# xinfushe/oclJPEGDecoder

Measured on NVIDIA B200. Metric: MPix/s decoded (1080p 4:2:0 q90 batch), higher is better.
Workload: dtype int32

## Files before the change

ocljpegdecoder_b200/csrc/b2j_internal.h:

```cpp
#ifndef B2J_INTERNAL_H_INCLUDED
#define B2J_INTERNAL_H_INCLUDED

#include <stdint.h>
#include <stddef.h>
#include <vector>

#include "../../include/b2j.h"

namespace b2j {

constexpr int kScanGroups = 4;
constexpr int kScanThreads = 256;
constexpr int kScanChunkBytes = kScanThreads * kScanGroups * 16;
constexpr int kHuffThreads = 128;
constexpr int kSubBytes = 128;
constexpr int kSyncPre = 2;
constexpr int kSyncLanes = kHuffThreads - kSyncPre;
constexpr int kLutBits = 10;
constexpr int kLutBitsDc = 6;
constexpr int kLutHeader = 16;
constexpr int kLutMaxDecode = 12288;
constexpr int kLutMaxEntries = 32768;
constexpr int kWalkBits = 10;
constexpr int kWalkBitsDc = 8;
// ... 26 lines not shown
    uint32_t has_dri;
    uint32_t width, height;
    uint32_t lut_off;
    uint32_t lut_len;
    uint32_t lut_dec_len;
    uint32_t mode;
    uint32_t tot_blks;
    uint32_t ny_blks;
    uint32_t nu_blks;
    uint32_t samp;
    uint32_t yh;
    uint32_t wide_q;
    uint32_t sub_first;
    uint32_t n_sub_max;
    uint32_t scta_first;
};

struct SubRec
{
    uint32_t p;
    uint32_t cz;
    uint32_t nblk;
    int32_t dc[3];
    uint32_t fs;
    uint32_t fc;
};
struct SubMid { uint32_t p, cz, nblk; int32_t dc[3]; uint32_t fs, fc; };
struct SubPre { uint32_t blk; int32_t dc[3]; };
constexpr uint32_t kSubInvalid = 0xFFFFFFFFu;
constexpr uint32_t kSubNone = 0xFFFFFFFFu;
// ... 23 lines not shown
```

ocljpegdecoder_b200/csrc/kernels.cu:

```cuda
#include <cuda.h>
#include <cuda_runtime.h>
#include <stdint.h>

#include "b2j_internal.h"
#include "b2j_math.h"
#include "b2j_sync.h"
#include "kernels.h"

namespace b2j {

__constant__ uint8_t c_zigzag2[64];

static const uint8_t h_zigzag[64] = B2J_ZIGZAG_TABLE;

cudaError_t init_constants()
{
    uint8_t z2[64];
    for (int i = 0; i < 64; i++) z2[i] = (uint8_t)(2 * h_zigzag[i]);
    return cudaMemcpyToSymbol(c_zigzag2, z2, sizeof(z2));
}

struct ScanFlags { uint32_t keep[4], mark[4], term[4]; };

constexpr uint32_t kFlagAll = 0x80808080u;

__device__ __forceinline__ uint32_t eq_ff(uint32_t w)
{
    return ((w & 0x7F7F7F7Fu) + 0x01010101u) & w & kFlagAll;
}
__device__ __forceinline__ void first_n_flags(int n, uint32_t m[4])
{
#pragma unroll
    for (int i = 0; i < 4; i++)
    {
// ... 174 lines not shown
        if (im.has_dri && rank + 1 < im.n_segs)
        {
            seg_start[im.seg_first + rank + 1] = clean_pos + __popc(keep16 & ((1u << j) - 1u));
            const uint32_t wj = j < 4u ? w[0] : (j < 8u ? w[1] : (j < 12u ? w[2] : w[3]));
            const uint32_t bj = (wj >> (8 * (j & 3u))) & 0xFFu;
            if (bj != 0xD0u + (rank & 7u)) atomicOr(&status[img_idx], B2J_ST_RST_MISMATCH);
        }
        rank++;
    }
}

constexpr int kScanMinCtas = 4;
__global__ void __launch_bounds__(kScanThreads, kScanMinCtas)
k_unstuff_fused(const uint8_t *__restrict__ raw, uint8_t *__restrict__ clean, const ImgDev *__restrict__ imgs,
                const uint32_t *__restrict__ chunk_img, uint64_t *__restrict__ chunk_state, uint32_t *__restrict__ clean_len,
                uint32_t *__restrict__ seg_start, int32_t *__restrict__ status)
{
    __shared__ uint32_t s_min;
    __shared__ uint32_t s_warp[kScanThreads / 32];
    __shared__ uint32_t s_base[3];
    __shared__ __align__(16) uint8_t s_out[kScanChunkBytes + 32];
    const uint32_t tid = threadIdx.x, lane = tid & 31, warp = tid >> 5;
    const uint32_t c = blockIdx.x;
    const uint32_t img_idx = chunk_img[c];
    const ImgDev &im = imgs[img_idx];
    const uint32_t k = c - im.chunk_first;
    const uint32_t pos = k * kScanChunkBytes + tid * (16u * kScanGroups);
    ScanThread st;
    st.load_classify(raw + im.raw_off, pos);
    uint32_t term = kNoTerm;
    {
        uint32_t any = 0;
#pragma unroll
        for (int g = 0; g < kScanGroups; g++) any |= st.f[g].term[0] | st.f[g].term[1] | st.f[g].term[2] | st.f[g].term[3];
        if (__syncthreads_or(any != 0u))
        {
            term = block_first_term(st.first_term(), tid, &s_min);
// ... 201 lines not shown
}

__device__ __forceinline__ int32_t extend_sz(uint32_t v, uint32_t size)
{
    const uint32_t u = __funnelshift_l(v, 0u, size);
    const uint32_t neg = (uint32_t)((int32_t)~v >> 31);
    return (int32_t)(u - __funnelshift_l(neg, 0u, size));
}

constexpr uint32_t kZzBytes = 192;
template <bool SYNC>
__global__ void __launch_bounds__(kHuffThreads)
k_huff_decode(const uint8_t *__restrict__ clean, const ImgDev *__restrict__ imgs, const HuffCtaDev *__restrict__ ctas,
              const uint32_t *__restrict__ seg_start, const uint32_t *__restrict__ clean_len,
              const uint16_t *__restrict__ luts, int16_t *__restrict__ coef, int32_t *__restrict__ status,
              const SubRec *__restrict__ recs, const uint4 *__restrict__ cta_base)
{
    extern __shared__ __align__(16) uint8_t smem[];
    uint8_t *s_slots = smem;
    uint8_t *s_zz2 = smem + kHuffThreads * 128;
    uint16_t *s_lut = reinterpret_cast<uint16_t *>(smem + kHuffThreads * 128 + kZzBytes);

    const uint32_t tid = threadIdx.x, lane = tid & 31;
    const HuffCtaDev cta = ctas[blockIdx.x];
    const ImgDev &im = imgs[cta.img];

    {
        const uint4 *src = reinterpret_cast<const uint4 *>(luts + im.lut_off);
        uint4 *dst = reinterpret_cast<uint4 *>(s_lut);
        for (uint32_t k = tid; k < im.lut_dec_len / 8; k += kHuffThreads) dst[k] = __ldg(src + k);
        uint4 *z = reinterpret_cast<uint4 *>(s_slots);
        for (uint32_t k = tid; k < kHuffThreads * 8; k += kHuffThreads) z[k] = make_uint4(0, 0, 0, 0);
        if (tid < 128) s_zz2[tid] = tid < 64 ? c_zigzag2[tid] : (uint8_t)0;
    }
    __syncthreads();

    const uint32_t tot = im.tot_blks, ny = im.ny_blks, nyu = im.ny_blks + im.nu_blks;
    const uint32_t seg = cta.seg_first + tid;
    uint32_t start = 0, end = 0, nblk = 0, blk0 = 0, start_bit = 0, bi = 0;
    int32_t dc0 = 0, dc1 = 0, dc2 = 0;
    int32_t err = 0;
    bool check_end = false, active, decodable;
    if (!SYNC)
    {
        active = seg < im.n_segs;
        if (active)
        {
            start = seg_start[im.seg_first + seg];
            const uint32_t mcu0 = seg * im.restart_interval;
            const uint32_t nmcu = min(im.restart_interval, im.mcu_count - mcu0);
            nblk = nmcu * tot;
            blk0 = im.blk_first + mcu0 * tot;
            if (seg + 1 < im.n_segs) { end = seg_start[im.seg_first + seg + 1]; check_end = (end != kSegInvalid); }
            if (!check_end) end = clean_len[cta.img];
        }
        decodable = active && start != kSegInvalid;
// ... 24 lines not shown
            for (int w = 0; w < kHuffThreads / 32; w++)
                if (w < (int)(tid >> 5)) { const uint4 t = s_wtot[w]; acc.x += t.x; acc.y += t.y; acc.z += t.z; acc.w += t.w; }
            pre.blk = acc.x + ib - rec.nblk;
            pre.dc[0] = (int32_t)acc.y + i0 - rec.dc[0]; pre.dc[1] = (int32_t)acc.z + i1 - rec.dc[1]; pre.dc[2] = (int32_t)acc.w + i2 - rec.dc[2];
        }
        if (active)
        {
            if (rec.fs != kSubNone && pre.blk < im.blk_count)
            {
                nblk = min(rec.nblk, im.blk_count - pre.blk);
                blk0 = im.blk_first + pre.blk;
                start_bit = rec.fs;
                bi = rec.fc;
                dc0 = pre.dc[0]; dc1 = pre.dc[1]; dc2 = pre.dc[2];
            }
            if (seg + 1 == n_sub && pre.blk + rec.nblk < im.blk_count) err |= B2J_ST_OVERRUN;
            end = clean_len[cta.img];
        }
        decodable = active && nblk > 0;
        {
            uint32_t *s_hist = reinterpret_cast<uint32_t *>(s_slots);
            uint32_t *s_wsum = s_hist + 640;
            uint32_t *s_desc = s_hist + 648;
            const uint32_t key = decodable ? bi * 64u + (63u - min(nblk, 63u)) : 639u;
            const uint32_t within = atomicAdd(&s_hist[key], 1u);
            __syncthreads();
            uint32_t h[5], sum = 0;
#pragma unroll
            for (int k = 0; k < 5; k++) { h[k] = s_hist[tid * 5u + k]; sum += h[k]; }
            uint32_t inc = sum;
#pragma unroll
            for (int o = 1; o < 32; o <<= 1)
            {
// ... 98 lines not shown
            {
                uint4 *sp = reinterpret_cast<uint4 *>(s_slots + warp_slot0 + j * 128u + ((ch ^ (j & 7u)) << 4));
                const uint4 v = *sp;
                *sp = make_uint4(0, 0, 0, 0);
                *reinterpret_cast<uint4 *>(coef + (size_t)dst * 64 + ch * 8) = v;
            }
        }
        __syncwarp();
        if (!SYNC && !dead)
        {
            const uint32_t nw_now = br.words_fetched();
            if (nw_now * 4u > seg_bytes + 16u) { err |= B2J_ST_OVERRUN; dead = true; }
        }
        bi = (bi + 1 == tot) ? 0u : bi + 1;
    }

    if (decodable && !dead)
    {
        const uint32_t nw = br.words_fetched();
        const uint64_t bits = (uint64_t)nw * 32u + br.bitpos - bit0;
        const uint64_t used = (bits + 7u) >> 3;
        const uint64_t avail = (uint64_t)end - start;
        if (used > avail) err |= B2J_ST_OVERRUN;
        else if (!SYNC && check_end && used != avail) err |= B2J_ST_SEGMENT_END;
    }
    if (err) atomicOr(&status[cta.img], err);
}

struct DevLut
{
// ... 86 lines not shown
        *chunk_state_k = make_uint4(sh.entry_used[kSyncPre].x, sh.entry_used[kSyncPre].y, sh.cur[last].p, sh.cur[last].cz);
    }
    __syncthreads();
}

__device__ __forceinline__ void sync_stage_lut(uint16_t *s_lut, const uint16_t *__restrict__ luts, const ImgDev &im)
{
    const uint4 *src = reinterpret_cast<const uint4 *>(luts + im.lut_off + im.lut_dec_len);
    uint4 *dst = reinterpret_cast<uint4 *>(s_lut);
    for (uint32_t k = threadIdx.x; k < (im.lut_len - im.lut_dec_len) / 8; k += kHuffThreads) dst[k] = __ldg(src + k);
}

__global__ void __launch_bounds__(kHuffThreads)
k_sync_chunks(const uint8_t *__restrict__ clean, const ImgDev *__restrict__ imgs, const HuffCtaDev *__restrict__ ctas,
              const uint32_t *__restrict__ clean_len, const uint16_t *__restrict__ luts, SubRec *__restrict__ recs,
              uint4 *__restrict__ chunk_state, uint4 *__restrict__ cta_tot, uint32_t *__restrict__ stats, uint32_t use_pre)
{
    extern __shared__ __align__(16) uint8_t smem[];
    __shared__ uint4 s_wtot[kHuffThreads / 32];
    __shared__ __align__(16) WalkCtab s_ctab[16];
    SyncShared &sh = *reinterpret_cast<SyncShared *>(smem);
    uint16_t *s_lut = reinterpret_cast<uint16_t *>(smem + kSyncSharedBytes);
    const HuffCtaDev cta = ctas[blockIdx.x];
    const ImgDev &im = imgs[cta.img];
    const uint32_t bits = clean_len[cta.img] * 8u;
    const uint32_t n_sub = (bits + kSubBytes * 8 - 1) / (kSubBytes * 8);
    if (cta.seg_first >= n_sub)
    {
        if (threadIdx.x == 0) { cta_tot[blockIdx.x] = make_uint4(0u, 0u, 0u, 0u); chunk_state[blockIdx.x] = make_uint4(0u, 0u, 0u, 0u); }
        return;
    }
    sync_stage_lut(s_lut, luts, im);
    __syncthreads();
    uint32_t sm_lut;
    asm volatile("mov.u32 %0, %1;" : "=r"(sm_lut) : "r"(smem_addr(smem) + kSyncSharedBytes));
    DevWalk wk;
    wk.init(clean + im.raw_off, sm_lut, luts + im.lut_off, s_ctab, im);
    __syncthreads();
    SyncChunk ch;
    ch.first = cta.seg_first; ch.n_sub = n_sub; ch.bits = bits;
    const bool pre = use_pre != 0u && cta.seg_first != 0u;
    ch.first_lane = pre ? (cta.seg_first >= (uint32_t)kSyncPre ? 0u : (uint32_t)kSyncPre - cta.seg_first) : (uint32_t)kSyncPre;
    ch.forced = cta.seg_first == 0u;
    ch.forced_entry = make_uint2(0u, 0u);
    sync_run_chunk(wk, sh, ch, recs + im.sub_first, chunk_state + blockIdx.x, cta_tot + blockIdx.x, stats, s_wtot);
}

// ... 539 lines not shown
    if (tid < n_mcus)
    {
        const uint32_t gm = d.mcu_first + tid;
        const uint32_t my = gm / mcu_count_w;
        sd.mcu_xy[tid] = make_uint2(gm - my * mcu_count_w, my);
    }
    if (tid == 0)
    {
        sd.pix = pix + pix_off;
        sd.width = width; sd.height = height;
        sd.mode = d.info & 0xFFu; sd.n_mcus = n_mcus;
        sd.samp = samp;
    }
}

template <bool NARROWQ>
__device__ __forceinline__ TileDev tile_load(TileSmem &sm, const CUtensorMap *tmap, const ImgDev *__restrict__ imgs, const TileDev *__restrict__ tiles,
                                             const uint16_t *__restrict__ qtabs, uint8_t *__restrict__ pix, int32_t *__restrict__ status)
{
    const uint32_t tid = threadIdx.x;
    const TileDev d = tiles[blockIdx.x];
    if (tid == 0)
    {
        mbar_init(&sm.bar, 1);
        asm volatile("fence.mbarrier_init.release.cluster;" ::: "memory");
        mbar_expect_tx(&sm.bar, kTileBlocks * 128);
        tma_load_2d(sm.tile, tmap, 0, (int)d.row_first, &sm.bar);
    }
    side_stage<NARROWQ>(sm.side, imgs, qtabs, d, pix);
    __syncthreads();
    uint32_t spins = 0;
    while (!mbar_try_wait(&sm.bar, 0))
    {
        if (++spins > (1u << 22)) { if (tid == 0) atomicOr(&status[d.img], B2J_ST_INTERNAL); break; }
    }
    return d;
}

constexpr int kIdctMinCtas = 5;
constexpr int kTileColour = 0, kTileGray = 1, kTileGeneric = 2;
template <bool NARROWQ, int FMT, int KIND>
__global__ void __launch_bounds__(kTileBlocks, kIdctMinCtas)
k_idct_csc(const __grid_constant__ CUtensorMap tmap, const ImgDev *__restrict__ imgs, const TileDev *__restrict__ tiles,
           const uint16_t *__restrict__ qtabs, uint8_t *__restrict__ pix, int32_t *__restrict__ status)
{
    TileSmem &sm = *tile_smem();
    const uint32_t tid = threadIdx.x;
    tile_load<NARROWQ>(sm, &tmap, imgs, tiles, qtabs, pix, status);
    if (KIND == kTileGray)
    {
        idct_phase<0, 0, NARROWQ>(sm.tile, sm.side);
        __syncthreads();
        csc_gray<FMT>(sm.tile, sm.side, tid);
    }
    else if (KIND == kTileGeneric)
    {
        idct_phase<-1, -1, NARROWQ>(sm.tile, sm.side);
        __syncthreads();
        csc_generic<FMT>(sm.tile, sm.side, tid);
    }
    else
    {
        idct_dispatch<NARROWQ>(sm.tile, sm.side);
// ... 142 lines not shown
    }
#pragma unroll
    for (int r = 0; r < 2; r++)
    {
        int64_t d[8], o[2];
#pragma unroll
        for (int c = 0; c < 8; c++) d[c] = ((kUsed >> c) & 1u) ? ws[r][c] : 0;
        red2_1d<13 + 2 + 3 + 2>(d, o);
        *reinterpret_cast<uint16_t *>(dst + (size_t)r * pitch) = (uint16_t)(islow_limit(o[0]) | islow_limit(o[1]) << 8);
    }
}

template <uint32_t MINS>
__global__ void __launch_bounds__(kTileBlocks)
k_idct_libjpeg(const __grid_constant__ CUtensorMap tmap, const ImgDev *__restrict__ imgs, const TileDev *__restrict__ tiles,
               const uint16_t *__restrict__ qtabs, uint8_t *__restrict__ samples, int32_t *__restrict__ status)
{
    TileSmem &sm = *tile_smem();
    const uint32_t tid = threadIdx.x;
    const TileDev d = tile_load<false>(sm, &tmap, imgs, tiles, qtabs, samples, status);
    const ImgDev *im = imgs + d.img;
    const uint32_t sp = sm.side.samp, n = sm.side.n_mcus;
    const uint32_t yh = sp & 15u, yv = (sp >> 4) & 15u, uh = (sp >> 8) & 15u, uv = (sp >> 12) & 15u, vh = (sp >> 16) & 15u, vv = (sp >> 20) & 15u;
    const uint32_t ny = yh * yv, nu = uh * uv, tot = ny + nu + vh * vv;
    if (tid >= n * tot) return;
    const uint32_t comp = (tid >= n * ny ? 1u : 0u) + (tid >= n * (ny + nu) ? 1u : 0u);
    const uint32_t before = (comp > 0 ? ny : 0u) + (comp > 1 ? nu : 0u);
    const uint32_t nc = comp == 0 ? ny : (comp == 1 ? nu : vh * vv);
    const uint32_t j = tid - n * before, m = j / nc, k = j % nc;
    const uint32_t h = comp == 0 ? yh : (comp == 1 ? uh : vh), v = comp == 0 ? yv : (comp == 1 ? uv : vv);
    const uint32_t ss = dct_size(h, v, yh, yv, MINS);
    const uint32_t mcu_count = __ldg(&im->mcu_count), mcw = __ldg(&im->mcu_count_w), blk_first = __ldg(&im->blk_first);
    const size_t pitch = (size_t)mcw * h * ss;
    const uint2 mxy = sm.side.mcu_xy[m];
    uint8_t *dst = samples + 64ull * ((size_t)blk_first + (size_t)mcu_count * before) + (size_t)((mxy.y * v + k / h) * ss) * pitch +
// ... 159 lines not shown

size_t huff_smem_bytes(uint32_t max_lut_len) { return (size_t)kHuffThreads * 128 + kZzBytes + (size_t)max_lut_len * 2; }

cudaError_t configure_kernels(uint32_t max_lut_len)
{
    const int hb = (int)huff_smem_bytes(kLutMaxDecode);
    cudaError_t e = cudaFuncSetAttribute(k_huff_decode<false>, cudaFuncAttributeMaxDynamicSharedMemorySize, hb);
    if (e != cudaSuccess) return e;
    e = cudaFuncSetAttribute(k_huff_decode<true>, cudaFuncAttributeMaxDynamicSharedMemorySize, hb);
    if (e != cudaSuccess) return e;
    e = cudaFuncSetAttribute(k_sync_chunks, cudaFuncAttributeMaxDynamicSharedMemorySize, (int)(kSyncSharedBytes + max_lut_len * 2));
    if (e != cudaSuccess) return e;
    return cudaFuncSetAttribute(k_sync_sweep, cudaFuncAttributeMaxDynamicSharedMemorySize, (int)(kSyncSharedBytes + max_lut_len * 2));
}

void launch_prepass(const DecodeArgs &a, cudaStream_t s)
{
    if (a.n_chunks == 0) return;
    k_unstuff_fused<<<a.n_chunks, kScanThreads, 0, s>>>(a.raw, a.clean, a.imgs, a.chunk_img, a.chunk_state, a.clean_len, a.seg_start, a.status);
}

void launch_huffman(const DecodeArgs &a, cudaStream_t s)
{
    if (a.n_huff_ctas == 0) return;
    k_huff_decode<false><<<a.n_huff_ctas, kHuffThreads, huff_smem_bytes(a.max_lut_dec_len), s>>>(a.clean, a.imgs, a.huff_ctas, a.seg_start, a.clean_len,
                                                                                                a.luts, a.coef, a.status, nullptr, nullptr);
}

void launch_huffman_sync(const DecodeArgs &a, cudaStream_t s)
{
    const uint32_t n = a.n_sync_ctas, ni = a.n_sync_imgs;
    if (n == 0 || ni == 0) return;
    const size_t sync_bytes = kSyncSharedBytes + (size_t)a.max_lut_walk_len * 2;
    k_sync_chunks<<<n, kHuffThreads, sync_bytes, s>>>(a.clean, a.imgs, a.sync_ctas, a.clean_len, a.luts, a.recs, a.sync_chunk_state, a.sync_cta_base,
                                                      a.sync_stats, a.sync_use_pre ? 1u : 0u);
    k_sync_sweep<<<ni, kHuffThreads, sync_bytes, s>>>(a.clean, a.imgs, a.sync_imgs, a.clean_len, a.luts, a.recs, a.sync_chunk_state, a.sync_cta_base,
                                                     a.sync_stats);
    k_sync_cta_scan<<<ni, 32, 0, s>>>(a.imgs, a.sync_imgs, a.sync_cta_base);
    k_huff_decode<true><<<n, kHuffThreads, huff_smem_bytes(a.max_lut_dec_len), s>>>(a.clean, a.imgs, a.sync_ctas, a.seg_start, a.clean_len, a.luts,
                                                                                    a.coef, a.status, a.recs, a.sync_cta_base);
}

template <int FMT, int KIND>
static void launch_idct_kind(const DecodeArgs &a, uint32_t first, uint32_t count, cudaStream_t s)
{
    if (count == 0) return;
    const auto kernel = a.any_wide_q ? k_idct_csc<false, FMT, KIND> : k_idct_csc<true, FMT, KIND>;
    kernel<<<count, kTileBlocks, kTileSmemBytes, s>>>(*a.tmap, a.imgs, a.tiles + first, a.qtabs, a.pixels, a.status);
}

template <int FMT>
static void launch_idct_format(const DecodeArgs &a, cudaStream_t s)
{
    launch_idct_kind<FMT, kTileColour>(a, 0, a.gray_tile0, s);
    launch_idct_kind<FMT, kTileGray>(a, a.gray_tile0, a.generic_tile0 - a.gray_tile0, s);
    launch_idct_kind<FMT, kTileGeneric>(a, a.generic_tile0, a.n_tiles - a.generic_tile0, s);
}

template <int FMT, uint32_t MINS>
static void launch_libjpeg_scale(const DecodeArgs &a, cudaStream_t s)
{
    const dim3 grid((a.max_px_groups + 255u) / 256u, a.n_images < 65535u ? a.n_images : 65535u);
    k_idct_libjpeg<MINS><<<a.n_tiles, kTileBlocks, kTileSmemBytes, s>>>(*a.tmap, a.imgs, a.tiles, a.qtabs, a.samples, a.status);
    k_upsample_libjpeg<FMT, MINS><<<grid, 256, 0, s>>>(a.samples, a.imgs, a.n_images, a.pixels);
}

template <int FMT>
static void launch_libjpeg_format(const DecodeArgs &a, cudaStream_t s)
{
    if (a.scale == 1) launch_libjpeg_scale<FMT, 8>(a, s);
    else if (a.scale == 2) launch_libjpeg_scale<FMT, 4>(a, s);
    else if (a.scale == 4) launch_libjpeg_scale<FMT, 2>(a, s);
    else launch_libjpeg_scale<FMT, 1>(a, s);
}

int idct_launches(const DecodeArgs &a)
{
    if (a.n_tiles == 0) return 0;
// ... 43 lines not shown
```

ocljpegdecoder_b200/csrc/kernels.h:

```cpp
#ifndef B2J_KERNELS_H_INCLUDED
#define B2J_KERNELS_H_INCLUDED

#include <cuda.h>
#include <cuda_runtime.h>
#include <stdint.h>

#include "b2j_internal.h"

namespace b2j {

struct DecodeArgs
{
    const uint8_t *raw;
    const ImgDev *imgs;
    const uint32_t *chunk_img;
    const HuffCtaDev *huff_ctas;
    const HuffCtaDev *sync_ctas;
    const uint32_t *sync_imgs;
    const TileDev *tiles;
    const uint16_t *luts;
    const uint16_t *qtabs;
    const CUtensorMap *tmap;
    uint8_t *clean;
    uint64_t *chunk_state;
    uint32_t *clean_len, *seg_start;
    SubRec *recs;
    uint4 *sync_cta_base;
    uint4 *sync_chunk_state;
    uint32_t *sync_stats;
    bool sync_use_pre;
    int16_t *coef;
    uint8_t *pixels;
    int32_t *status;
    uint32_t n_images, n_chunks, n_huff_ctas, n_sync_ctas, n_sync_imgs, max_lut_len, max_lut_dec_len, max_lut_walk_len;
    uint32_t gray_tile0, generic_tile0, n_tiles;
    int out_format;
    bool any_wide_q;
    int pixel_model;
    uint8_t *samples;
    uint32_t max_px_groups;
    uint32_t scale;
};

cudaError_t init_constants();
// ... 16 lines not shown
```

ocljpegdecoder_b200/csrc/runtime.cu:

```cuda
#include <cuda.h>
#include <cuda_runtime.h>
#include <cudaTypedefs.h>

#include <stdio.h>
#include <stdlib.h>
#include <string.h>
#include <fcntl.h>
#include <sys/stat.h>
#include <unistd.h>

#include <algorithm>
#include <atomic>
#include <condition_variable>
#include <map>
#include <mutex>
#include <thread>
#include <string>
#include <vector>

#include "b2j_internal.h"
#include "b2j_math.h"
#include "kernels.h"

using namespace b2j;
// ... 79 lines not shown
    std::vector<ImgDev> imgs;
    b2j_batch_info info;

    PoolBuf h_blob, d_blob;
    size_t blob_bytes;
    ImgDev *h_imgs;

    PoolBuf d_scratch, d_coef, d_pix;
    size_t clean_bytes;
    size_t zero_bytes;
    size_t coef_rows;
    uint32_t n_segs_total;
    PoolBuf d_expand;
    PoolBuf d_small;
    PoolBuf d_samples;
    int small_factor = 0;
    std::vector<uint64_t> small_off;

    CUtensorMap tmap;
    DecodeArgs args;
    bool uploaded = false;
    cudaStream_t last_stream = nullptr;
};

namespace {

int make_tensor_map(b2j_ctx *ctx, b2j_batch *b)
{
    memset(&b->tmap, 0, sizeof(b->tmap));
    const cuuint64_t dims[2] = {64, (cuuint64_t)b->coef_rows};
// ... 56 lines not shown
cudaError_t grow(b2j_ctx *ctx, PoolBuf &buf, size_t n)
{
    if (buf.cap >= n) return cudaSuccess;
    std::lock_guard<std::mutex> lk(ctx->mu);
    ctx->dev_pool.put(buf);
    const cudaError_t e = ctx->dev_pool.get(n, buf);
    if (e != cudaSuccess) cudaGetLastError();
    return e;
}

void release_batch_buffers(b2j_batch *b)
{
    b2j_ctx *c = b->ctx;
    std::lock_guard<std::mutex> lk(c->mu);
    c->pin_pool.put(b->h_blob);
    for (PoolBuf *d : {&b->d_blob, &b->d_scratch, &b->d_coef, &b->d_pix, &b->d_expand, &b->d_small, &b->d_samples}) c->dev_pool.put(*d);
}

int64_t device_bytes(const b2j_batch *b)
{
    return (int64_t)(b->d_blob.cap + b->d_scratch.cap + b->d_coef.cap + b->d_pix.cap + b->d_samples.cap);
}

const ImgDev *image_of(const b2j_batch *b, int image) { return b && image >= 0 && image < b->n ? &b->imgs[(size_t)image] : nullptr; }

size_t format_bpp(int fmt) { return fmt == B2J_OUT_BGRA ? 4 : 3; }

uint32_t out_width(const b2j_batch *b, const ImgDev &im) { return (im.width + b->args.scale - 1) / b->args.scale; }
uint32_t out_height(const b2j_batch *b, const ImgDev &im) { return (im.height + b->args.scale - 1) / b->args.scale; }

size_t image_bytes(const b2j_batch *b, const ImgDev &im) { return (size_t)out_width(b, im) * out_height(b, im) * format_bpp(b->args.out_format); }
// ... 235 lines not shown
            const uint32_t off = (uint32_t)luts.size();
            luts.insert(luts.end(), set.begin(), set.end());
            it = lut_cache.emplace(key, LutRef{off, (uint32_t)set.size(), (uint32_t)set[12]}).first;
        }
        im.lut_off = it->second.off;
        im.lut_len = it->second.len;
        im.lut_dec_len = it->second.dec_len;
        if (im.lut_len > max_lut_len) max_lut_len = im.lut_len;
        if (im.lut_dec_len > max_lut_dec_len) max_lut_dec_len = im.lut_dec_len;
        if (im.lut_len - im.lut_dec_len > max_lut_walk_len) max_lut_walk_len = im.lut_len - im.lut_dec_len;
    }
    if (rc != B2J_OK) { delete b; return rc; }
    if (blk_total + kTileBlocks >= 0xFFFFFFF0ull) { delete b; return B2J_E_ARG; }
    const auto gray0 = std::stable_partition(tiles.begin(), tiles.end(), [](const TileDev &t) { return (t.info & 0xFFu) < kModeGray; });
    const auto generic0 = std::stable_partition(gray0, tiles.end(), [](const TileDev &t) { return (t.info & 0xFFu) == kModeGray; });

    size_t off = 0;
    auto place = [&](size_t bytes) { const size_t o = off; off = align_up(off + bytes, 256); return o; };
    auto place_array = [&](const auto &v) { return place(sizeof(v[0]) * v.size()); };
    const size_t o_imgs = place_array(b->imgs);
    const size_t o_chunk_img = place_array(chunk_img);
    const size_t o_ctas = place_array(ctas);
    const size_t o_sctas = place_array(sctas);
    const size_t o_simgs = place_array(simgs);
    const size_t o_tiles = place_array(tiles);
    const size_t o_luts = place_array(luts);
    const size_t o_qtabs = place_array(qtabs);
    const size_t o_raw = place(raw_total + kScanChunkBytes + 64);
    b->blob_bytes = off;

    off = 0;
    const size_t o_clean = place(raw_total + 256);
    b->clean_bytes = off - o_clean;
    const size_t o_clean_len = place(4 * (size_t)n);
    const size_t o_seg_start = place(4 * (size_t)seg_total);
    const size_t o_recs = place(sizeof(SubRec) * (size_t)sub_total);
    const size_t o_pres = place(sizeof(uint4) * (sctas.size() + 1));
    const size_t o_chunk_states = place(sizeof(uint4) * (sctas.size() + 1));
    const size_t o_status = place(4 * (size_t)n);
    const size_t o_sync_stats = place(4 * 8);
    const size_t o_chunk_state = place(8 * chunk_img.size());
    b->zero_bytes = off - o_status;
    const size_t scratch_bytes = off;
    b->n_segs_total = seg_total;
    b->coef_rows = blk_total + kTileBlocks;

    {
        std::lock_guard<std::mutex> lk(ctx->mu);
        cudaError_t e;
        if ((e = ctx->pin_pool.get(b->blob_bytes, b->h_blob)) != cudaSuccess ||
            (e = ctx->dev_pool.get(b->blob_bytes, b->d_blob)) != cudaSuccess ||
            (e = ctx->dev_pool.get(scratch_bytes, b->d_scratch)) != cudaSuccess ||
            (e = ctx->dev_pool.get(b->coef_rows * 128, b->d_coef)) != cudaSuccess ||
            (e = ctx->dev_pool.get(pix_total, b->d_pix)) != cudaSuccess)
        {
            rc = fail_cuda(e, "batch allocation");
// ... 20 lines not shown
        uint8_t *dst = at<uint8_t>(b->h_blob, o_raw + im.raw_off);
        if (im.raw_len) memcpy(dst, files[i] + descs[i].scan_offset, im.raw_len);
        memset(dst + im.raw_len, 0xD9, align_up((size_t)im.raw_len + 32, 16) - im.raw_len);
        dst[im.raw_len] = 0xFF;
    }
    a.raw = at<const uint8_t>(b->d_blob, o_raw);
    a.clean = at<uint8_t>(b->d_scratch, o_clean);
    a.clean_len = at<uint32_t>(b->d_scratch, o_clean_len);
    a.seg_start = at<uint32_t>(b->d_scratch, o_seg_start);
    a.recs = at<SubRec>(b->d_scratch, o_recs);
    a.sync_cta_base = at<uint4>(b->d_scratch, o_pres);
    a.sync_chunk_state = at<uint4>(b->d_scratch, o_chunk_states);
    a.status = at<int32_t>(b->d_scratch, o_status);
    a.sync_stats = at<uint32_t>(b->d_scratch, o_sync_stats);
    a.chunk_state = at<uint64_t>(b->d_scratch, o_chunk_state);
    a.tmap = &b->tmap;
    a.coef = at<int16_t>(b->d_coef, 0);
    a.pixels = at<uint8_t>(b->d_pix, 0);
    a.n_images = (uint32_t)n;
    a.n_chunks = (uint32_t)chunk_img.size();
    a.n_huff_ctas = (uint32_t)ctas.size();
    a.n_sync_ctas = (uint32_t)sctas.size();
    a.n_sync_imgs = (uint32_t)simgs.size();
    a.gray_tile0 = (uint32_t)(gray0 - tiles.begin());
    a.generic_tile0 = (uint32_t)(generic0 - tiles.begin());
    a.n_tiles = (uint32_t)tiles.size();
    a.max_lut_len = max_lut_len;
    a.max_lut_dec_len = max_lut_dec_len;
    a.max_lut_walk_len = max_lut_walk_len;
    a.out_format = B2J_OUT_BGRA;
// ... 44 lines not shown
extern "C" int b2j_batch_upload(b2j_batch *b, void *stream)
{
    if (!b) return B2J_E_ARG;
    CU_TRY(cudaSetDevice(b->ctx->device));
    cudaStream_t s = pick_stream(b, stream);
    CU_TRY(cudaMemcpyAsync(b->d_blob.p, b->h_blob.p, b->blob_bytes, cudaMemcpyHostToDevice, s));
    if (!b->uploaded)
    {
        CU_TRY(cudaMemsetAsync(b->args.coef + (b->coef_rows - kTileBlocks) * 64, 0, (size_t)kTileBlocks * 128, s));
        CU_TRY(cudaMemsetAsync(b->args.clean, 0, b->clean_bytes, s));
        b->uploaded = true;
    }
    return B2J_OK;
}

constexpr size_t kStepEvents = 5;

static int enqueue_decode(b2j_batch *b, cudaStream_t s, cudaEvent_t *ev )
{
    if (!b->uploaded) { t_last_error = "b2j_batch_decode before b2j_batch_upload"; return B2J_E_ARG; }
    if (b->args.scale != 1 && b->args.pixel_model != B2J_PIXELS_LIBJPEG)
    {
        t_last_error = "a scaled decode (b2j_batch_set_scale) needs the libjpeg pixel model: the reference has none";
        return B2J_E_ARG;
    }
    if (b->args.pixel_model == B2J_PIXELS_LIBJPEG && !b->d_samples.p)
    {
        const cudaError_t e = grow(b->ctx, b->d_samples, (size_t)b->info.total_blocks * 64);
        if (e != cudaSuccess) { fail_cuda(e, "sample plane allocation"); return B2J_E_NOMEM; }
        b->args.samples = at<uint8_t>(b->d_samples, 0);
        b->info.device_bytes = device_bytes(b);
    }
    const DecodeArgs &a = b->args;
    if (ev) CU_TRY(cudaEventRecord(ev[0], s));
    if (a.n_huff_ctas) CU_TRY(cudaMemsetAsync(a.seg_start, 0xFF, 4 * (size_t)b->n_segs_total, s));
    CU_TRY(cudaMemsetAsync(a.status, 0, b->zero_bytes, s));
    if (ev) CU_TRY(cudaEventRecord(ev[1], s));
    launch_prepass(a, s);
    if (ev) CU_TRY(cudaEventRecord(ev[2], s));
    launch_huffman(a, s);
    launch_huffman_sync(a, s);
    if (ev) CU_TRY(cudaEventRecord(ev[3], s));
    launch_idct(a, s);
    if (ev) CU_TRY(cudaEventRecord(ev[4], s));
    CU_TRY(cudaGetLastError());
    return B2J_OK;
}

static void collect_times(cudaEvent_t *ev, b2j_stage_times *t)
{
    t->prepass_ms = t->huffman_ms = t->idct_ms = 0.f;
    cudaEventElapsedTime(&t->prepass_ms, ev[1], ev[2]);
    cudaEventElapsedTime(&t->huffman_ms, ev[2], ev[3]);
    cudaEventElapsedTime(&t->idct_ms, ev[3], ev[4]);
    cudaEventElapsedTime(&t->total_ms, ev[0], ev[4]);
}

extern "C" int b2j_batch_decode(b2j_batch *b, void *stream)
{
    if (!b) return B2J_E_ARG;
    CU_TRY(cudaSetDevice(b->ctx->device));
    return enqueue_decode(b, pick_stream(b, stream), nullptr);
}

extern "C" int b2j_batch_decode_timed(b2j_batch *b, void *stream, b2j_stage_times *times)
{
    return b2j_batch_decode_steps(b, stream, 1, times, nullptr);
}

extern "C" int b2j_batch_decode_steps(b2j_batch *b, void *stream, int steps, b2j_stage_times *per_step, float *total_ms)
{
    if (!b || steps <= 0) return B2J_E_ARG;
    CU_TRY(cudaSetDevice(b->ctx->device));
    cudaStream_t s = pick_stream(b, stream);
    const size_t per = kStepEvents;
    std::vector<cudaEvent_t> ev((size_t)steps * per, nullptr);
    int rc = B2J_OK;
    for (auto &e : ev)
    {
        const cudaError_t ce = cudaEventCreate(&e);
        if (ce != cudaSuccess) { rc = fail_cuda(ce, "cudaEventCreate"); e = nullptr; break; }
    }
    for (int k = 0; k < steps && rc == B2J_OK; k++) rc = enqueue_decode(b, s, &ev[(size_t)k * per]);
    if (rc == B2J_OK)
    {
        cudaError_t e = cudaStreamSynchronize(s);
        if (e != cudaSuccess) rc = fail_cuda(e, "cudaStreamSynchronize");
    }
    if (rc == B2J_OK)
    {
        for (int k = 0; k < steps && per_step; k++) collect_times(&ev[(size_t)k * per], &per_step[k]);
        if (total_ms) cudaEventElapsedTime(total_ms, ev[0], ev[(size_t)steps * per - 1]);
    }
    for (auto &e : ev) if (e) cudaEventDestroy(e);
    return rc;
}

extern "C" int b2j_batch_sync(b2j_batch *b, void *stream)
{
    if (!b) return B2J_E_ARG;
    CU_TRY(cudaSetDevice(b->ctx->device));
    CU_TRY(cudaStreamSynchronize(pick_stream(b, stream)));
    return B2J_OK;
}

extern "C" int b2j_batch_status(b2j_batch *b, void *stream, int32_t *status)
// ... 593 lines not shown
```

Baseline: 341,600.

## Overlap Huffman decode and IDCT via PDL and per-tile readiness counters

Adds programmatic dependent launch (griddepcontrol) so the Huffman and IDCT kernels can launch early and stage LUTs and zigzag tables before waiting on the previous kernel. Huffman CTAs atomically credit per-tile ready counters after writing coefficients. IDCT CTAs spin on those counters with acquire loads and a timeout before issuing their TMA load, instead of waiting for the whole Huffman grid to finish. Stage timing moves from events between kernels to device globaltimer stamps. The risks are spin-wait overhead, CTAs occupying SMs while waiting (possible starvation or deadlock guarded only by the timeout), and extra atomics.

```diff
diff --git a/ocljpegdecoder_b200/csrc/b2j_internal.h b/ocljpegdecoder_b200/csrc/b2j_internal.h
--- a/ocljpegdecoder_b200/csrc/b2j_internal.h
+++ b/ocljpegdecoder_b200/csrc/b2j_internal.h
@@ -64,6 +64,7 @@
     uint32_t sub_first;
     uint32_t n_sub_max;
     uint32_t scta_first;
+    uint32_t tile_first;
 };
 
 struct SubRec
diff --git a/ocljpegdecoder_b200/csrc/kernels.cu b/ocljpegdecoder_b200/csrc/kernels.cu
--- a/ocljpegdecoder_b200/csrc/kernels.cu
+++ b/ocljpegdecoder_b200/csrc/kernels.cu
@@ -18,6 +18,28 @@
     uint8_t z2[64];
     for (int i = 0; i < 64; i++) z2[i] = (uint8_t)(2 * h_zigzag[i]);
     return cudaMemcpyToSymbol(c_zigzag2, z2, sizeof(z2));
+}
+
+__device__ __forceinline__ void pdl_launch_dependents() { asm volatile("griddepcontrol.launch_dependents;" ::: "memory"); }
+__device__ __forceinline__ void pdl_wait() { asm volatile("griddepcontrol.wait;" ::: "memory"); }
+
+__device__ __forceinline__ uint64_t global_ns()
+{
+    uint64_t t;
+    asm volatile("mov.u64 %0, %%globaltimer;" : "=l"(t));
+    return t;
+}
+__device__ __forceinline__ void clock_first(uint64_t *c, int i) { if (c) atomicMax(reinterpret_cast<unsigned long long *>(c + i), ~global_ns()); }
+__device__ __forceinline__ void clock_last(uint64_t *c, int i) { if (c) atomicMax(reinterpret_cast<unsigned long long *>(c + i), global_ns()); }
+
+__device__ __forceinline__ void credit_tiles(uint32_t *__restrict__ ready, uint32_t b0, uint32_t n, uint32_t bpt)
+{
+    for (uint32_t b = b0, e = b0 + n; b < e;)
+    {
+        const uint32_t t = b / bpt, te = min((t + 1u) * bpt, e);
+        atomicAdd(ready + t, te - b);
+        b = te;
+    }
 }
 
 struct ScanFlags { uint32_t keep[4], mark[4], term[4]; };
@@ -222,13 +244,15 @@
 __global__ void __launch_bounds__(kScanThreads, kScanMinCtas)
 k_unstuff_fused(const uint8_t *__restrict__ raw, uint8_t *__restrict__ clean, const ImgDev *__restrict__ imgs,
                 const uint32_t *__restrict__ chunk_img, uint64_t *__restrict__ chunk_state, uint32_t *__restrict__ clean_len,
-                uint32_t *__restrict__ seg_start, int32_t *__restrict__ status)
+                uint32_t *__restrict__ seg_start, int32_t *__restrict__ status, uint64_t *clock)
 {
     __shared__ uint32_t s_min;
     __shared__ uint32_t s_warp[kScanThreads / 32];
     __shared__ uint32_t s_base[3];
     __shared__ __align__(16) uint8_t s_out[kScanChunkBytes + 32];
     const uint32_t tid = threadIdx.x, lane = tid & 31, warp = tid >> 5;
+    pdl_launch_dependents();
+    if (tid == 0) clock_first(clock, 0);
     const uint32_t c = blockIdx.x;
     const uint32_t img_idx = chunk_img[c];
     const ImgDev &im = imgs[img_idx];
@@ -460,7 +484,7 @@
 k_huff_decode(const uint8_t *__restrict__ clean, const ImgDev *__restrict__ imgs, const HuffCtaDev *__restrict__ ctas,
               const uint32_t *__restrict__ seg_start, const uint32_t *__restrict__ clean_len,
               const uint16_t *__restrict__ luts, int16_t *__restrict__ coef, int32_t *__restrict__ status,
-              const SubRec *__restrict__ recs, const uint4 *__restrict__ cta_base)
+              const SubRec *__restrict__ recs, const uint4 *__restrict__ cta_base, uint32_t *__restrict__ tile_ready, uint64_t *clock)
 {
     extern __shared__ __align__(16) uint8_t smem[];
     uint8_t *s_slots = smem;
@@ -468,6 +492,7 @@
     uint16_t *s_lut = reinterpret_cast<uint16_t *>(smem + kHuffThreads * 128 + kZzBytes);
 
     const uint32_t tid = threadIdx.x, lane = tid & 31;
+    pdl_launch_dependents();
     const HuffCtaDev cta = ctas[blockIdx.x];
     const ImgDev &im = imgs[cta.img];
 
@@ -479,6 +504,8 @@
         for (uint32_t k = tid; k < kHuffThreads * 8; k += kHuffThreads) z[k] = make_uint4(0, 0, 0, 0);
         if (tid < 128) s_zz2[tid] = tid < 64 ? c_zigzag2[tid] : (uint8_t)0;
     }
+    pdl_wait();
+    if (tid == 0) clock_first(clock, 1);
     __syncthreads();
 
     const uint32_t tot = im.tot_blks, ny = im.ny_blks, nyu = im.ny_blks + im.nu_blks;
@@ -486,6 +513,7 @@
     uint32_t start = 0, end = 0, nblk = 0, blk0 = 0, start_bit = 0, bi = 0;
     int32_t dc0 = 0, dc1 = 0, dc2 = 0;
     int32_t err = 0;
+    uint32_t miss0 = 0, miss_n = 0;
     bool check_end = false, active, decodable;
     if (!SYNC)
     {
@@ -540,9 +568,15 @@
                 bi = rec.fc;
                 dc0 = pre.dc[0]; dc1 = pre.dc[1]; dc2 = pre.dc[2];
             }
-            if (seg + 1 == n_sub && pre.blk + rec.nblk < im.blk_count) err |= B2J_ST_OVERRUN;
+            if (seg + 1 == n_sub && pre.blk + rec.nblk < im.blk_count)
+            {
+                err |= B2J_ST_OVERRUN;
+                miss0 = pre.blk + rec.nblk;
+                miss_n = im.blk_count - miss0;
+            }
             end = clean_len[cta.img];
         }
+        else if (n_sub == 0 && seg == 0) miss_n = im.blk_count;
         decodable = active && nblk > 0;
         {
             uint32_t *s_hist = reinterpret_cast<uint32_t *>(s_slots);
@@ -671,6 +705,15 @@
         }
         bi = (bi + 1 == tot) ? 0u : bi + 1;
     }
+    if (tile_ready)
+    {
+        __threadfence();
+        __syncwarp();
+        const uint32_t bpt = kTileBlocks / tot * tot;
+        credit_tiles(tile_ready + im.tile_first, blk0 - im.blk_first, nblk, bpt);
+        if (SYNC) credit_tiles(tile_ready + im.tile_first, miss0, miss_n, bpt);
+    }
+    if (lane == 0) clock_last(clock, 2);
 
     if (decodable && !dead)
     {
@@ -787,7 +830,7 @@
 __global__ void __launch_bounds__(kHuffThreads)
 k_sync_chunks(const uint8_t *__restrict__ clean, const ImgDev *__restrict__ imgs, const HuffCtaDev *__restrict__ ctas,
               const uint32_t *__restrict__ clean_len, const uint16_t *__restrict__ luts, SubRec *__restrict__ recs,
-              uint4 *__restrict__ chunk_state, uint4 *__restrict__ cta_tot, uint32_t *__restrict__ stats, uint32_t use_pre)
+              uint4 *__restrict__ chunk_state, uint4 *__restrict__ cta_tot, uint32_t *__restrict__ stats, uint32_t use_pre, uint64_t *clock)
 {
     extern __shared__ __align__(16) uint8_t smem[];
     __shared__ uint4 s_wtot[kHuffThreads / 32];
@@ -796,6 +839,9 @@
     uint16_t *s_lut = reinterpret_cast<uint16_t *>(smem + kSyncSharedBytes);
     const HuffCtaDev cta = ctas[blockIdx.x];
     const ImgDev &im = imgs[cta.img];
+    sync_stage_lut(s_lut, luts, im);
+    pdl_wait();
+    if (threadIdx.x == 0) clock_first(clock, 1);
     const uint32_t bits = clean_len[cta.img] * 8u;
     const uint32_t n_sub = (bits + kSubBytes * 8 - 1) / (kSubBytes * 8);
     if (cta.seg_first >= n_sub)
@@ -803,7 +849,6 @@
         if (threadIdx.x == 0) { cta_tot[blockIdx.x] = make_uint4(0u, 0u, 0u, 0u); chunk_state[blockIdx.x] = make_uint4(0u, 0u, 0u, 0u); }
         return;
     }
-    sync_stage_lut(s_lut, luts, im);
     __syncthreads();
     uint32_t sm_lut;
     asm volatile("mov.u32 %0, %1;" : "=r"(sm_lut) : "r"(smem_addr(smem) + kSyncSharedBytes));
@@ -1373,9 +1418,27 @@
     }
 }
 
+constexpr uint64_t kTileWaitNs = 2000000000ull;
+__device__ __forceinline__ void tile_wait(const uint32_t *ready, uint32_t *abandon, uint32_t need, int32_t *status)
+{
+    uint32_t v, ns = 32;
+    const uint64_t t0 = global_ns();
+    while (true)
+    {
+        asm volatile("ld.acquire.gpu.global.u32 %0, [%1];" : "=r"(v) : "l"(ready) : "memory");
+        if (v >= need) break;
+        if (*reinterpret_cast<volatile uint32_t *>(abandon)) break;
+        if (global_ns() - t0 > kTileWaitNs) { atomicOr(status, B2J_ST_INTERNAL); atomicExch(abandon, 1u); break; }
+        __nanosleep(ns);
+        ns = ns < 512u ? 2u * ns : ns;
+    }
+    asm volatile("fence.proxy.async.global;" ::: "memory");
+}
+
 template <bool NARROWQ>
 __device__ __forceinline__ TileDev tile_load(TileSmem &sm, const CUtensorMap *tmap, const ImgDev *__restrict__ imgs, const TileDev *__restrict__ tiles,
-                                             const uint16_t *__restrict__ qtabs, uint8_t *__restrict__ pix, int32_t *__restrict__ status)
+                                             const uint32_t *ready, uint32_t *abandon, const uint16_t *__restrict__ qtabs,
+                                             uint8_t *__restrict__ pix, int32_t *__restrict__ status)
 {
     const uint32_t tid = threadIdx.x;
     const TileDev d = tiles[blockIdx.x];
@@ -1383,6 +1446,7 @@
     {
         mbar_init(&sm.bar, 1);
         asm volatile("fence.mbarrier_init.release.cluster;" ::: "memory");
+        if (ready) tile_wait(ready + blockIdx.x, abandon, (d.info >> 8) * __ldg(&imgs[d.img].tot_blks), status + d.img);
         mbar_expect_tx(&sm.bar, kTileBlocks * 128);
         tma_load_2d(sm.tile, tmap, 0, (int)d.row_first, &sm.bar);
     }
@@ -1401,11 +1465,11 @@
 template <bool NARROWQ, int FMT, int KIND>
 __global__ void __launch_bounds__(kTileBlocks, kIdctMinCtas)
 k_idct_csc(const __grid_constant__ CUtensorMap tmap, const ImgDev *__restrict__ imgs, const TileDev *__restrict__ tiles,
-           const uint16_t *__restrict__ qtabs, uint8_t *__restrict__ pix, int32_t *__restrict__ status)
+           const uint32_t *ready, uint32_t *abandon, const uint16_t *__restrict__ qtabs, uint8_t *__restrict__ pix, int32_t *__restrict__ status)
 {
     TileSmem &sm = *tile_smem();
     const uint32_t tid = threadIdx.x;
-    tile_load<NARROWQ>(sm, &tmap, imgs, tiles, qtabs, pix, status);
+    tile_load<NARROWQ>(sm, &tmap, imgs, tiles, ready, abandon, qtabs, pix, status);
     if (KIND == kTileGray)
     {
         idct_phase<0, 0, NARROWQ>(sm.tile, sm.side);
@@ -1578,11 +1642,12 @@
 template <uint32_t MINS>
 __global__ void __launch_bounds__(kTileBlocks)
 k_idct_libjpeg(const __grid_constant__ CUtensorMap tmap, const ImgDev *__restrict__ imgs, const TileDev *__restrict__ tiles,
-               const uint16_t *__restrict__ qtabs, uint8_t *__restrict__ samples, int32_t *__restrict__ status)
+               const uint32_t *ready, uint32_t *abandon, const uint16_t *__restrict__ qtabs, uint8_t *__restrict__ samples,
+               int32_t *__restrict__ status)
 {
     TileSmem &sm = *tile_smem();
     const uint32_t tid = threadIdx.x;
-    const TileDev d = tile_load<false>(sm, &tmap, imgs, tiles, qtabs, samples, status);
+    const TileDev d = tile_load<false>(sm, &tmap, imgs, tiles, ready, abandon, qtabs, samples, status);
     const ImgDev *im = imgs + d.img;
     const uint32_t sp = sm.side.samp, n = sm.side.n_mcus;
     const uint32_t yh = sp & 15u, yv = (sp >> 4) & 15u, uh = (sp >> 8) & 15u, uv = (sp >> 12) & 15u, vh = (sp >> 16) & 15u, vv = (sp >> 20) & 15u;
@@ -1772,17 +1837,30 @@
     return cudaFuncSetAttribute(k_sync_sweep, cudaFuncAttributeMaxDynamicSharedMemorySize, (int)(kSyncSharedBytes + max_lut_len * 2));
 }
 
+template <typename... P, typename... A>
+static void launch_ex(void (*kernel)(P...), dim3 grid, dim3 block, size_t smem, cudaStream_t s, bool dependent, A... args)
+{
+    cudaLaunchAttribute attr[1];
+    attr[0].id = cudaLaunchAttributeProgrammaticStreamSerialization;
+    attr[0].val.programmaticStreamSerializationAllowed = 1;
+    cudaLaunchConfig_t cfg = {};
+    cfg.gridDim = grid; cfg.blockDim = block; cfg.dynamicSmemBytes = smem; cfg.stream = s;
+    cfg.attrs = attr; cfg.numAttrs = dependent ? 1 : 0;
+    cudaLaunchKernelEx(&cfg, kernel, static_cast<P>(args)...);
+}
+
 void launch_prepass(const DecodeArgs &a, cudaStream_t s)
 {
     if (a.n_chunks == 0) return;
-    k_unstuff_fused<<<a.n_chunks, kScanThreads, 0, s>>>(a.raw, a.clean, a.imgs, a.chunk_img, a.chunk_state, a.clean_len, a.seg_start, a.status);
+    k_unstuff_fused<<<a.n_chunks, kScanThreads, 0, s>>>(a.raw, a.clean, a.imgs, a.chunk_img, a.chunk_state, a.clean_len, a.seg_start, a.status,
+                                                         a.clock);
 }
 
 void launch_huffman(const DecodeArgs &a, cudaStream_t s)
 {
     if (a.n_huff_ctas == 0) return;
-    k_huff_decode<false><<<a.n_huff_ctas, kHuffThreads, huff_smem_bytes(a.max_lut_dec_len), s>>>(a.clean, a.imgs, a.huff_ctas, a.seg_start, a.clean_len,
-                                                                                                a.luts, a.coef, a.status, nullptr, nullptr);
+    launch_ex(k_huff_decode<false>, a.n_huff_ctas, kHuffThreads, huff_smem_bytes(a.max_lut_dec_len), s, true, a.clean, a.imgs, a.huff_ctas,
+              a.seg_start, a.clean_len, a.luts, a.coef, a.status, (const SubRec *)nullptr, (const uint4 *)nullptr, a.tile_ready, a.clock);
 }
 
 void launch_huffman_sync(const DecodeArgs &a, cudaStream_t s)
@@ -1790,13 +1868,13 @@
     const uint32_t n = a.n_sync_ctas, ni = a.n_sync_imgs;
     if (n == 0 || ni == 0) return;
     const size_t sync_bytes = kSyncSharedBytes + (size_t)a.max_lut_walk_len * 2;
-    k_sync_chunks<<<n, kHuffThreads, sync_bytes, s>>>(a.clean, a.imgs, a.sync_ctas, a.clean_len, a.luts, a.recs, a.sync_chunk_state, a.sync_cta_base,
-                                                      a.sync_stats, a.sync_use_pre ? 1u : 0u);
+    launch_ex(k_sync_chunks, n, kHuffThreads, sync_bytes, s, a.n_huff_ctas == 0, a.clean, a.imgs, a.sync_ctas, a.clean_len, a.luts, a.recs,
+              a.sync_chunk_state, a.sync_cta_base, a.sync_stats, a.sync_use_pre ? 1u : 0u, a.clock);
     k_sync_sweep<<<ni, kHuffThreads, sync_bytes, s>>>(a.clean, a.imgs, a.sync_imgs, a.clean_len, a.luts, a.recs, a.sync_chunk_state, a.sync_cta_base,
                                                      a.sync_stats);
     k_sync_cta_scan<<<ni, 32, 0, s>>>(a.imgs, a.sync_imgs, a.sync_cta_base);
     k_huff_decode<true><<<n, kHuffThreads, huff_smem_bytes(a.max_lut_dec_len), s>>>(a.clean, a.imgs, a.sync_ctas, a.seg_start, a.clean_len, a.luts,
-                                                                                    a.coef, a.status, a.recs, a.sync_cta_base);
+                                                                                    a.coef, a.status, a.recs, a.sync_cta_base, a.tile_ready, a.clock);
 }
 
 template <int FMT, int KIND>
@@ -1804,7 +1882,8 @@
 {
     if (count == 0) return;
     const auto kernel = a.any_wide_q ? k_idct_csc<false, FMT, KIND> : k_idct_csc<true, FMT, KIND>;
-    kernel<<<count, kTileBlocks, kTileSmemBytes, s>>>(*a.tmap, a.imgs, a.tiles + first, a.qtabs, a.pixels, a.status);
+    launch_ex(kernel, count, kTileBlocks, kTileSmemBytes, s, a.tile_ready && first == 0, *a.tmap, a.imgs, a.tiles + first,
+              a.tile_ready ? a.tile_ready + first : nullptr, a.tile_ready ? a.tile_ready + a.n_tiles : nullptr, a.qtabs, a.pixels, a.status);
 }
 
 template <int FMT>
@@ -1819,7 +1898,8 @@
 static void launch_libjpeg_scale(const DecodeArgs &a, cudaStream_t s)
 {
     const dim3 grid((a.max_px_groups + 255u) / 256u, a.n_images < 65535u ? a.n_images : 65535u);
-    k_idct_libjpeg<MINS><<<a.n_tiles, kTileBlocks, kTileSmemBytes, s>>>(*a.tmap, a.imgs, a.tiles, a.qtabs, a.samples, a.status);
+    launch_ex(k_idct_libjpeg<MINS>, a.n_tiles, kTileBlocks, kTileSmemBytes, s, a.tile_ready != nullptr, *a.tmap, a.imgs, a.tiles, a.tile_ready,
+              a.tile_ready ? a.tile_ready + a.n_tiles : nullptr, a.qtabs, a.samples, a.status);
     k_upsample_libjpeg<FMT, MINS><<<grid, 256, 0, s>>>(a.samples, a.imgs, a.n_images, a.pixels);
 }
 
diff --git a/ocljpegdecoder_b200/csrc/kernels.h b/ocljpegdecoder_b200/csrc/kernels.h
--- a/ocljpegdecoder_b200/csrc/kernels.h
+++ b/ocljpegdecoder_b200/csrc/kernels.h
@@ -28,6 +28,8 @@
     uint4 *sync_cta_base;
     uint4 *sync_chunk_state;
     uint32_t *sync_stats;
+    uint32_t *tile_ready;
+    uint64_t *clock;
     bool sync_use_pre;
     int16_t *coef;
     uint8_t *pixels;
diff --git a/ocljpegdecoder_b200/csrc/runtime.cu b/ocljpegdecoder_b200/csrc/runtime.cu
--- a/ocljpegdecoder_b200/csrc/runtime.cu
+++ b/ocljpegdecoder_b200/csrc/runtime.cu
@@ -117,6 +117,7 @@
     PoolBuf d_expand;
     PoolBuf d_small;
     PoolBuf d_samples;
+    PoolBuf d_clock;
     int small_factor = 0;
     std::vector<uint64_t> small_off;
 
@@ -203,7 +204,7 @@
     b2j_ctx *c = b->ctx;
     std::lock_guard<std::mutex> lk(c->mu);
     c->pin_pool.put(b->h_blob);
-    for (PoolBuf *d : {&b->d_blob, &b->d_scratch, &b->d_coef, &b->d_pix, &b->d_expand, &b->d_small, &b->d_samples}) c->dev_pool.put(*d);
+    for (PoolBuf *d : {&b->d_blob, &b->d_scratch, &b->d_coef, &b->d_pix, &b->d_expand, &b->d_small, &b->d_samples, &b->d_clock}) c->dev_pool.put(*d);
 }
 
 int64_t device_bytes(const b2j_batch *b)
@@ -469,6 +470,8 @@
     if (blk_total + kTileBlocks >= 0xFFFFFFF0ull) { delete b; return B2J_E_ARG; }
     const auto gray0 = std::stable_partition(tiles.begin(), tiles.end(), [](const TileDev &t) { return (t.info & 0xFFu) < kModeGray; });
     const auto generic0 = std::stable_partition(gray0, tiles.end(), [](const TileDev &t) { return (t.info & 0xFFu) == kModeGray; });
+    for (size_t t = 0; t < tiles.size(); t++)
+        if (tiles[t].mcu_first == 0) b->imgs[tiles[t].img].tile_first = (uint32_t)t;
 
     size_t off = 0;
     auto place = [&](size_t bytes) { const size_t o = off; off = align_up(off + bytes, 256); return o; };
@@ -495,6 +498,7 @@
     const size_t o_status = place(4 * (size_t)n);
     const size_t o_sync_stats = place(4 * 8);
     const size_t o_chunk_state = place(8 * chunk_img.size());
+    const size_t o_tile_ready = place(4 * (tiles.size() + 1));
     b->zero_bytes = off - o_status;
     const size_t scratch_bytes = off;
     b->n_segs_total = seg_total;
@@ -545,6 +549,8 @@
     a.status = at<int32_t>(b->d_scratch, o_status);
     a.sync_stats = at<uint32_t>(b->d_scratch, o_sync_stats);
     a.chunk_state = at<uint64_t>(b->d_scratch, o_chunk_state);
+    a.tile_ready = coef_only ? nullptr : at<uint32_t>(b->d_scratch, o_tile_ready);
+    a.clock = nullptr;
     a.tmap = &b->tmap;
     a.coef = at<int16_t>(b->d_coef, 0);
     a.pixels = at<uint8_t>(b->d_pix, 0);
@@ -619,9 +625,10 @@
     return B2J_OK;
 }
 
-constexpr size_t kStepEvents = 5;
-
-static int enqueue_decode(b2j_batch *b, cudaStream_t s, cudaEvent_t *ev )
+constexpr size_t kStepEvents = 3;
+constexpr size_t kStepClock = 4;
+
+static int enqueue_decode(b2j_batch *b, cudaStream_t s, cudaEvent_t *ev , uint64_t *clock )
 {
     if (!b->uploaded) { t_last_error = "b2j_batch_decode before b2j_batch_upload"; return B2J_E_ARG; }
     if (b->args.scale != 1 && b->args.pixel_model != B2J_PIXELS_LIBJPEG)
@@ -636,36 +643,39 @@
         b->args.samples = at<uint8_t>(b->d_samples, 0);
         b->info.device_bytes = device_bytes(b);
     }
-    const DecodeArgs &a = b->args;
+    DecodeArgs a = b->args;
+    a.clock = clock;
     if (ev) CU_TRY(cudaEventRecord(ev[0], s));
     if (a.n_huff_ctas) CU_TRY(cudaMemsetAsync(a.seg_start, 0xFF, 4 * (size_t)b->n_segs_total, s));
     CU_TRY(cudaMemsetAsync(a.status, 0, b->zero_bytes, s));
     if (ev) CU_TRY(cudaEventRecord(ev[1], s));
     launch_prepass(a, s);
-    if (ev) CU_TRY(cudaEventRecord(ev[2], s));
     launch_huffman(a, s);
     launch_huffman_sync(a, s);
-    if (ev) CU_TRY(cudaEventRecord(ev[3], s));
     launch_idct(a, s);
-    if (ev) CU_TRY(cudaEventRecord(ev[4], s));
+    if (ev) CU_TRY(cudaEventRecord(ev[2], s));
     CU_TRY(cudaGetLastError());
     return B2J_OK;
 }
 
-static void collect_times(cudaEvent_t *ev, b2j_stage_times *t)
-{
-    t->prepass_ms = t->huffman_ms = t->idct_ms = 0.f;
-    cudaEventElapsedTime(&t->prepass_ms, ev[1], ev[2]);
-    cudaEventElapsedTime(&t->huffman_ms, ev[2], ev[3]);
-    cudaEventElapsedTime(&t->idct_ms, ev[3], ev[4]);
-    cudaEventElapsedTime(&t->total_ms, ev[0], ev[4]);
+static void collect_times(cudaEvent_t *ev, const uint64_t *clock, b2j_stage_times *t)
+{
+    float span = 0.f;
+    cudaEventElapsedTime(&span, ev[1], ev[2]);
+    cudaEventElapsedTime(&t->total_ms, ev[0], ev[2]);
+    const uint64_t p0 = ~clock[0], h0 = ~clock[1], h1 = clock[2];
+    const bool ok = clock[0] && clock[1] && h1 > h0 && h0 > p0;
+    constexpr float kMin = 1e-4f;
+    t->prepass_ms = ok ? (float)((h0 - p0) * 1e-6) : kMin;
+    t->huffman_ms = ok ? (float)((h1 - h0) * 1e-6) : kMin;
+    t->idct_ms = std::max(span - t->prepass_ms - t->huffman_ms, kMin);
 }
 
 extern "C" int b2j_batch_decode(b2j_batch *b, void *stream)
 {
     if (!b) return B2J_E_ARG;
     CU_TRY(cudaSetDevice(b->ctx->device));
-    return enqueue_decode(b, pick_stream(b, stream), nullptr);
+    return enqueue_decode(b, pick_stream(b, stream), nullptr, nullptr);
 }
 
 extern "C" int b2j_batch_decode_timed(b2j_batch *b, void *stream, b2j_stage_times *times)
@@ -679,6 +689,13 @@
     CU_TRY(cudaSetDevice(b->ctx->device));
     cudaStream_t s = pick_stream(b, stream);
     const size_t per = kStepEvents;
+    const size_t clock_bytes = (size_t)steps * kStepClock * 8;
+    {
+        const cudaError_t e = grow(b->ctx, b->d_clock, clock_bytes);
+        if (e != cudaSuccess) { fail_cuda(e, "stage clock allocation"); return B2J_E_NOMEM; }
+    }
+    uint64_t *clock = at<uint64_t>(b->d_clock, 0);
+    CU_TRY(cudaMemsetAsync(clock, 0, clock_bytes, s));
     std::vector<cudaEvent_t> ev((size_t)steps * per, nullptr);
     int rc = B2J_OK;
     for (auto &e : ev)
@@ -686,15 +703,21 @@
         const cudaError_t ce = cudaEventCreate(&e);
         if (ce != cudaSuccess) { rc = fail_cuda(ce, "cudaEventCreate"); e = nullptr; break; }
     }
-    for (int k = 0; k < steps && rc == B2J_OK; k++) rc = enqueue_decode(b, s, &ev[(size_t)k * per]);
+    for (int k = 0; k < steps && rc == B2J_OK; k++) rc = enqueue_decode(b, s, &ev[(size_t)k * per], clock + (size_t)k * kStepClock);
     if (rc == B2J_OK)
     {
         cudaError_t e = cudaStreamSynchronize(s);
         if (e != cudaSuccess) rc = fail_cuda(e, "cudaStreamSynchronize");
     }
+    std::vector<uint64_t> h_clock((size_t)steps * kStepClock);
+    if (rc == B2J_OK && per_step)
+    {
+        const cudaError_t e = cudaMemcpy(h_clock.data(), clock, clock_bytes, cudaMemcpyDeviceToHost);
+        if (e != cudaSuccess) rc = fail_cuda(e, "stage clock read-back");
+    }
     if (rc == B2J_OK)
     {
-        for (int k = 0; k < steps && per_step; k++) collect_times(&ev[(size_t)k * per], &per_step[k]);
+        for (int k = 0; k < steps && per_step; k++) collect_times(&ev[(size_t)k * per], &h_clock[(size_t)k * kStepClock], &per_step[k]);
         if (total_ms) cudaEventElapsedTime(total_ms, ev[0], ev[(size_t)steps * per - 1]);
     }
     for (auto &e : ev) if (e) cudaEventDestroy(e);
```

Result: slower. 316,400 (median of 6 runs) (-7.4%).
